# luo-ziyuan/NeRF_Signature

Measured on AMD Instinct MI355X. Metric: training rays/sec @4096 rays (hotdog, 32-bit msg), higher is better.
Workload: dtype f32 (hash gather, compositing) + fp16 MFMA with f32 accumulate (MLPs)

## Files before the change

include/nerfsig.h:

```cpp
#ifndef NERFSIG_H_
#define NERFSIG_H_

#include <stddef.h>
#include <stdint.h>

#ifdef __cplusplus
extern "C" {
#endif

#define NSIG_OK 0
#define NSIG_ERR_ARG 1
#define NSIG_ERR_LAUNCH 2

#define NSIG_TABLE_ROWS (1u << 19)
#define NSIG_BASE_LEVELS 16
#define NSIG_MAX_MESSAGE_DIM 64

typedef void *nsig_stream_t;

int nsig_abi_version(void);
const char *nsig_last_error(void);


int rm_near_far_from_aabb(const float *rays_o, const float *rays_d, const float *aabb, uint32_t N, float min_near,
// ... 164 lines not shown
int opt_adam_dense(uint32_t n, float *const *params_host, const float *const *grads_host, float *const *exp_avg_host,
                   float *const *exp_avg_sq_host, float *const *steps_host, const uint32_t *numel_host, const float *lr, float beta1,
                   float beta2, float eps, float grad_scale, float *scratch, nsig_stream_t stream);
int opt_adam_dense_host(uint32_t n, float *const *params_host, const float *const *grads_host, float *const *exp_avg_host,
                        float *const *exp_avg_sq_host, const uint32_t *numel_host, const float *step_sizes_host, const float *inv_bc2_host,
                        float beta1, float beta2, float eps, float grad_scale, nsig_stream_t stream);

int rm_composite_train_finish_fwd(const float *sigmas, const float *rgbs, const float *deltas, const int32_t *rays, uint32_t M, uint32_t N,
                                  float T_thresh, const float *nears, const float *fars, const float *bg, uint32_t bg_stride,
                                  float *weights_sum, float *depth, float *image, float *image_out, float *depth_out, nsig_stream_t stream);
int rm_composite_train_finish_bwd(const float *grad_weights_sum, const float *grad_image_out, const float *sigmas, const float *rgbs,
                                  const float *deltas, const int32_t *rays, const float *weights_sum, const float *image, const float *bg,
                                  uint32_t bg_stride, uint32_t M, uint32_t N, float T_thresh, uint32_t rays_in_order, float *grad_sigmas,
                                  float *grad_rgbs, nsig_stream_t stream);


int rm_finish_fwd(const float *image, const float *depth, const float *weights_sum, const float *nears, const float *fars, const float *bg,
                  uint32_t bg_stride, uint32_t N, float *image_out, float *depth_out, nsig_stream_t stream);
int rm_finish_bwd(const float *grad_image, const float *grad_depth, const float *depth, const float *nears, const float *fars, const float *bg,
                  uint32_t bg_stride, uint32_t N, float *grad_weights_sum, float *grad_depth_in, nsig_stream_t stream);

int loop_step_begin(float *G, uint32_t n_floats, const float *ring_dev, uint32_t slots, uint32_t width, uint32_t *counter, float *msg,
                    nsig_stream_t stream);
void *nsig_host_device_pointer(const void *pinned_host);

int wm_loss_fwd(const float *content, const float *gt, uint32_t n_content, const float *decoded, const float *message, uint32_t D, float temp,
                float lambda_w, float lambda_i, float *losses3, float *d_content, float *d_decoded, nsig_stream_t stream);
int wm_loss_bwd(const float *g_lossi, const float *g_lossw, const float *g_loss, float lambda_w, float lambda_i, const float *d_content,
                uint32_t n_content, const float *d_decoded, uint32_t D, float *grad_content, float *grad_decoded, nsig_stream_t stream);


int dec_bn_gelu_fwd(const float *x, const float *gamma, const float *beta, uint32_t N, uint32_t C, uint32_t P, float eps, float *y,
                    float *save, nsig_stream_t stream);
int dec_bn_gelu_bwd(const float *dy, const float *x, const float *gamma, const float *beta, const float *save, uint32_t N, uint32_t C,
                    uint32_t P, float *dx, float *dgamma, float *dbeta, nsig_stream_t stream);

size_t dec_workspace_bytes(uint32_t B, uint32_t Cin, uint32_t H, uint32_t W);
int dec_forward(const float *img, uint32_t input_mode, const float *mean_host, const float *std_host, const float *const *params_host,
                uint32_t B, uint32_t Cin, uint32_t H, uint32_t W, float eps, void *workspace, float *decoded, float *clamped_out,
                nsig_stream_t stream);
int dec_backward(const float *grad_decoded, const float *img, uint32_t input_mode, const float *mean_host, const float *std_host,
                 const float *const *params_host, uint32_t B, uint32_t Cin, uint32_t H, uint32_t W, void *workspace,
                 float *const *grads_host, float *grad_img, nsig_stream_t stream, nsig_stream_t weights_stream);

int dec_forward_train(const float *img, const float *mean_host, const float *std_host, const float *const *params_host, uint32_t B,
                      uint32_t Cin, uint32_t H, uint32_t W, float eps, void *workspace, float *decoded, float *clamped_out,
// ... 74 lines not shown
```

nerf_signature_amd/_native.py:

```python
import ctypes
import os

import torch

_PKG = os.path.dirname(os.path.abspath(__file__))
LIB_PATH = os.path.join(_PKG, "lib", "libnerfsig.so")

_c = ctypes
_vp, _u32, _fl, _int, _sz = _c.c_void_p, _c.c_uint32, _c.c_float, _c.c_int, _c.c_size_t

SIGNATURES = {
    "nsig_abi_version": [],
    "nsig_last_error": [],
    "nsig_host_device_pointer": [_vp],
    "rg_sample_rays": [_vp, _u32, _vp, _fl, _fl, _fl, _fl, _u32, _u32, _u32, _vp, _u32, _u32, _c.c_uint64, _vp, _vp, _vp, _vp, _vp, _vp],
    "rg_get_rays": [_vp, _fl, _fl, _fl, _fl, _u32, _u32, _vp, _u32, _u32, _vp, _vp, _vp],
    "rm_near_far_from_aabb": [_vp, _vp, _vp, _u32, _fl, _vp, _vp, _vp],
    "rm_sph_from_ray": [_vp, _vp, _fl, _u32, _vp, _vp],
    "rm_morton3D": [_vp, _u32, _vp, _vp],
    "rm_morton3D_invert": [_vp, _u32, _vp, _vp],
    "rm_packbits": [_vp, _u32, _fl, _vp, _vp],
    "rg_refresh_draw_scratch_bytes": [_u32, _u32],
    "rg_refresh_begin": [_vp, _u32, _vp],
    "rg_refresh_draw": [_vp, _vp, _u32, _u32, _vp, _vp, _c.c_uint64, _vp, _u32, _vp],
# ... 32 lines not shown
    "hg_level_lookup": [_vp, _u32, _fl, _vp, _vp, _vp],
    "opt_codebook_adam": [_vp, _vp, _vp, _vp, _u32, _fl, _fl, _fl, _vp, _vp, _fl, _vp],
    "opt_codebook_adam_sel": [_vp, _vp, _vp, _vp, _vp, _vp, _u32, _vp, _fl, _fl, _fl, _fl, _vp, _vp],
    "opt_codebook_adam_sel_next": [_vp, _vp, _vp, _vp, _vp, _vp, _u32, _vp, _fl, _fl, _fl, _fl, _vp, _vp, _vp, _vp],
    "mlp_packed_bytes": [],
    "mlp_get_precision": [],
    "mlp_set_precision": [_int],
    "mlp_get_pipelined": [],
    "mlp_set_pipelined": [_int],
    "mlp_pack_weights": [_vp, _vp, _vp, _vp],
    "hg_planes_bytes": [_u32],
    "hg_encode_planes": [_vp, _u32, _fl, _vp, _vp, _vp, _vp],
    "hg_warm_tables": [_vp, _vp, _vp, _vp],
    "hg_encode_codebook_plane": [_vp, _u32, _fl, _vp, _vp, _int, _vp, _vp],
    "field_fwd": [_vp, _vp, _u32, _fl, _vp, _vp, _vp, _vp, _vp, _vp, _vp, _vp, _int, _vp],
    "field_color_fwd": [_vp, _vp, _u32, _vp, _vp, _vp],
    "opt_adam_dense_host": [_u32, _vp, _vp, _vp, _vp, _vp, _vp, _vp, _fl, _fl, _fl, _fl, _vp],
    "opt_adam_dense": [_u32, _vp, _vp, _vp, _vp, _vp, _vp, _vp, _fl, _fl, _fl, _fl, _vp, _vp],
    "rm_composite_train_finish_fwd": [_vp, _vp, _vp, _vp, _u32, _u32, _fl, _vp, _vp, _vp, _u32, _vp, _vp, _vp, _vp, _vp, _vp],
    "rm_composite_train_finish_bwd": [_vp, _vp, _vp, _vp, _vp, _vp, _vp, _vp, _vp, _u32, _u32, _u32, _fl, _u32, _vp, _vp, _vp],
    "rm_finish_fwd": [_vp, _vp, _vp, _vp, _vp, _vp, _u32, _u32, _vp, _vp, _vp],
    "rm_finish_bwd": [_vp, _vp, _vp, _vp, _vp, _vp, _u32, _u32, _vp, _vp, _vp],
    "loop_step_begin": [_vp, _u32, _vp, _u32, _u32, _vp, _vp, _vp],
    "wm_loss_fwd": [_vp, _vp, _u32, _vp, _vp, _u32, _fl, _fl, _fl, _vp, _vp, _vp, _vp],
    "wm_loss_bwd": [_vp, _vp, _vp, _fl, _fl, _vp, _u32, _vp, _u32, _vp, _vp, _vp],
    "dec_bn_gelu_fwd": [_vp, _vp, _vp, _u32, _u32, _u32, _fl, _vp, _vp, _vp],
    "dec_bn_gelu_bwd": [_vp, _vp, _vp, _vp, _vp, _u32, _u32, _u32, _vp, _vp, _vp, _vp],
    "dec_workspace_bytes": [_u32, _u32, _u32, _u32],
    "dec_forward": [_vp, _u32, _vp, _vp, _vp, _u32, _u32, _u32, _u32, _fl, _vp, _vp, _vp, _vp],
    "dec_backward": [_vp, _vp, _u32, _vp, _vp, _vp, _u32, _u32, _u32, _u32, _vp, _vp, _vp, _vp, _vp],
    "dec_forward_train": [_vp, _vp, _vp, _vp, _u32, _u32, _u32, _u32, _fl, _vp, _vp, _vp, _u32, _vp, _vp, _vp, _fl, _fl, _vp, _vp],
    "dec_backward_train": [_vp, _vp, _vp, _vp, _vp, _u32, _u32, _u32, _u32, _vp, _vp, _vp, _u32, _vp, _vp, _vp, _vp, _vp],
    "wm_distort_draw": [_u32, _c.c_uint64, _vp, _u32, _vp, _vp, _vp],
    "wm_distort_fwd": [_vp, _u32, _u32, _u32, _u32, _u32, _vp, _vp, _vp, _vp],
    "wm_distort_bwd": [_vp, _vp, _u32, _u32, _u32, _u32, _u32, _vp, _vp, _vp, _vp],
    "wm_distort_geom_fwd": [_vp, _u32, _u32, _u32, _u32, _u32, _vp, _u32, _vp, _vp, _vp],
    "wm_distort_geom_bwd": [_vp, _vp, _u32, _u32, _u32, _u32, _u32, _vp, _u32, _vp, _vp],
    "field_fwd_trace": [_vp, _vp, _u32, _fl, _vp, _vp, _vp, _vp, _vp, _vp, _vp, _vp, _vp, _vp, _vp],
    "field_bwd_trace": [_u32, _vp, _vp, _vp, _vp, _vp, _vp, _vp, _vp, _vp, _vp, _vp, _vp, _vp],
    "hg_scatter_level": [_vp, _fl, _vp, _u32, _u32, _vp, _vp],
    "hg_scatter_binned_scratch_bytes": [_u32],
    "hg_scatter_binned": [_vp, _u32, _vp, _vp, _vp],
    "hg_scatter_levels_scratch_bytes": [_u32],
    "hg_scatter_levels": [_vp, _fl, _vp, _u32, _u32, _vp, _vp, _vp],
    "field_bwd": [_vp, _u32, _fl, _vp, _vp, _vp, _vp, _vp, _vp, _vp, _vp, _vp, _vp],
    "field_bwd_planned": [_vp, _u32, _fl, _vp, _vp, _vp, _vp, _vp, _vp, _vp, _vp],
    "hg_scatter_plan_bytes": [_u32],
    "hg_scatter_plan": [_vp, _u32, _fl, _vp, _vp],
    "hg_scatter_planned": [_vp, _u32, _vp, _vp],
    "field_fwd_trace_rows": [_vp, _vp, _u32, _vp, _fl, _vp, _vp, _vp, _vp, _vp, _vp, _vp, _vp, _vp, _vp, _vp],
    "field_fwd_trace_f16": [_vp, _vp, _u32, _vp, _fl, _vp, _vp, _vp, _vp, _vp, _vp, _vp, _vp, _vp, _vp, _vp],
    "field_bwd_trace_rows": [_u32, _vp, _vp, _vp, _vp, _vp, _vp, _vp, _vp, _vp, _vp, _vp, _vp, _vp, _vp],
    "field_wgrad_scratch_bytes": [_u32],
    "field_wgrad": [_u32, _vp, _vp, _vp, _vp, _vp, _vp, _vp, _vp, _vp, _vp, _vp, _vp, _vp, _vp, _vp],
    "field_bwd_wgrad_scratch_bytes": [_u32],
    "field_bwd_wgrad": [_u32, _vp, _vp, _vp, _vp, _vp, _vp, _vp, _vp, _vp, _vp, _vp, _vp, _vp, _vp, _vp, _vp, _vp],
    "field_bwd_wgrad_f16": [_u32, _vp, _vp, _vp, _vp, _vp, _vp, _vp, _vp, _vp, _vp, _vp, _vp, _vp, _vp, _vp, _vp, _vp],
    "rm_composite_train_mse": [_vp, _vp, _vp, _vp, _u32, _u32, _fl, _vp, _vp, _vp, _u32, _vp, _u32, _fl, _vp, _vp, _vp, _vp, _vp, _vp, _vp, _vp, _vp],
    "opt_ema_update": [_u32, _vp, _vp, _vp, _vp, _c.c_double, _vp],
    "clean_loss": [_vp, _vp, _u32, _fl, _vp, _vp, _vp, _vp, _vp, _vp, _u32, _vp, _u32, _c.c_uint64, _vp],
    "hg_levels_plan_bytes": [_u32],
    "hg_levels_plan": [_vp, _u32, _vp, _fl, _vp, _vp],
    "hg_levels_scatter": [_vp, _u32, _vp, _fl, _vp, _u32, _vp, _vp, _vp],
    "hg_levels_scatter_adam": [_vp, _u32, _vp, _fl, _vp, _u32, _vp, _vp, _vp, _vp, _vp, _vp, _fl, _fl, _fl, _fl, _vp, _vp],
}
_RESTYPES = {"nsig_last_error": _c.c_char_p, "nsig_host_device_pointer": _c.c_void_p, "rm_march_train_scratch_bytes": _sz, "mlp_packed_bytes": _sz, "hg_planes_bytes": _sz, "dec_workspace_bytes": _sz, "hg_scatter_levels_scratch_bytes": _sz, "hg_scatter_binned_scratch_bytes": _sz, "hg_scatter_plan_bytes": _sz, "field_wgrad_scratch_bytes": _sz, "field_bwd_wgrad_scratch_bytes": _sz, "hg_levels_plan_bytes": _sz, "rg_refresh_partials_bytes": _sz, "rg_refresh_draw_scratch_bytes": _sz}

_lib = None


class NativeError(RuntimeError):
    pass


def load():
    global _lib
    if _lib is not None:
        return _lib
    path = os.environ.get("NERFSIG_LIB", LIB_PATH)
    if not os.path.exists(path):
        raise NativeError(f"{path} not found: the HIP extension is required (no fallback). "
                          f"Build it with `python -m nerf_signature_amd.build`.")
    _lib = ctypes.CDLL(path)
    _lib.nsig_last_error.restype = _c.c_char_p
    return _lib


_bound = {}

# ... 71 lines not shown
```

nerf_signature_amd/csrc/hashgrid.hip:

```cpp
#include <cstdlib>
#include "hashgrid.h"

namespace nsig {

__global__ void __launch_bounds__(256) k_codebook_presum(CodebookPtrs tabs, uint32_t D, float4 *__restrict__ S) {
    const uint32_t e = blockIdx.x * blockDim.x + threadIdx.x;
    if (e >= NSIG_TABLE_ROWS / 2) return;
    float4 acc = {0.f, 0.f, 0.f, 0.f};
    uint32_t i = 0;
    for (; i + 4 <= D; i += 4) {
        const float4 a = reinterpret_cast<const float4 *>(tabs.p[i])[e];
        const float4 b = reinterpret_cast<const float4 *>(tabs.p[i + 1])[e];
        const float4 c = reinterpret_cast<const float4 *>(tabs.p[i + 2])[e];
        const float4 d = reinterpret_cast<const float4 *>(tabs.p[i + 3])[e];
        acc.x = (((acc.x + a.x) + b.x) + c.x) + d.x;
        acc.y = (((acc.y + a.y) + b.y) + c.y) + d.y;
        acc.z = (((acc.z + a.z) + b.z) + c.z) + d.z;
        acc.w = (((acc.w + a.w) + b.w) + c.w) + d.w;
    }
    for (; i < D; ++i) {
        const float4 a = reinterpret_cast<const float4 *>(tabs.p[i])[e];
        acc.x += a.x; acc.y += a.y; acc.z += a.z; acc.w += a.w;
    }
    S[e] = acc;
// ... 935 lines not shown
    const float step = *sp + 1.0f;
    *sp = step;
    scratch[i] = (float)((double)*lr / (1.0 - exp((double)step * log((double)beta1))));
    scratch[D + i] = (float)(1.0 / sqrt(1.0 - exp((double)step * log((double)beta2))));
}

typedef float nsig_f32x4 __attribute__((ext_vector_type(4)));
template <bool NT>
__device__ __forceinline__ float4 ld4(const float4 *p) {
    if (!NT) return *p;
    const nsig_f32x4 v = __builtin_nontemporal_load(reinterpret_cast<const nsig_f32x4 *>(p));
    return make_float4(v.x, v.y, v.z, v.w);
}
template <bool NT>
__device__ __forceinline__ void st4(float4 *p, const float4 &a) {
    if (!NT) {
        *p = a;
        return;
    }
    const nsig_f32x4 v = {a.x, a.y, a.z, a.w};
    __builtin_nontemporal_store(v, reinterpret_cast<nsig_f32x4 *>(p));
}

template <bool NEXT, bool NT>
__global__ void __launch_bounds__(256) k_codebook_adam_sel(const float4 *__restrict__ G, AdamPairPtrs a, const float *__restrict__ message,
                                                           const float *__restrict__ scratch, uint32_t D, float beta1, float beta2, float eps,
                                                           float grad_scale, const float *__restrict__ next_message, float4 *__restrict__ S_next) {
    const uint32_t e = blockIdx.x * blockDim.x + threadIdx.x;
    if (e >= NSIG_TABLE_ROWS / 2) return;
    float4 g = ld4<NT>(G + e);
    g.x *= grad_scale; g.y *= grad_scale; g.z *= grad_scale; g.w *= grad_scale;
    float4 acc = {0.f, 0.f, 0.f, 0.f};
    const float4 zero = {0.f, 0.f, 0.f, 0.f};
    uint32_t i = 0;
    for (; i + 2 <= D; i += 2) {
        const uint32_t j0 = 2 * i + (message[i] != 0.0f), j1 = 2 * i + 2 + (message[i + 1] != 0.0f);
        float4 *pp0 = reinterpret_cast<float4 *>(a.p[j0]) + e, *pm0 = reinterpret_cast<float4 *>(a.m[j0]) + e, *pv0 = reinterpret_cast<float4 *>(a.v[j0]) + e;
        float4 *pp1 = reinterpret_cast<float4 *>(a.p[j1]) + e, *pm1 = reinterpret_cast<float4 *>(a.m[j1]) + e, *pv1 = reinterpret_cast<float4 *>(a.v[j1]) + e;
        bool other0 = false, other1 = false;
        float4 o0 = zero, o1 = zero;
        if (NEXT) {
            other0 = (next_message[i] != 0.0f) != (message[i] != 0.0f);
            other1 = (next_message[i + 1] != 0.0f) != (message[i + 1] != 0.0f);
            if (other0) o0 = ld4<NT>(reinterpret_cast<const float4 *>(a.p[j0 ^ 1u]) + e);
            if (other1) o1 = ld4<NT>(reinterpret_cast<const float4 *>(a.p[j1 ^ 1u]) + e);
        }
        float4 p0 = ld4<NT>(pp0), m0 = ld4<NT>(pm0), v0 = ld4<NT>(pv0), p1 = ld4<NT>(pp1), m1 = ld4<NT>(pm1), v1 = ld4<NT>(pv1);
        const float ss0 = scratch[i], ib0 = scratch[D + i], ss1 = scratch[i + 1], ib1 = scratch[D + i + 1];
        adam_update(g.x, p0.x, m0.x, v0.x, beta1, beta2, eps, ss0, ib0);
        adam_update(g.y, p0.y, m0.y, v0.y, beta1, beta2, eps, ss0, ib0);
        adam_update(g.z, p0.z, m0.z, v0.z, beta1, beta2, eps, ss0, ib0);
        adam_update(g.w, p0.w, m0.w, v0.w, beta1, beta2, eps, ss0, ib0);
        adam_update(g.x, p1.x, m1.x, v1.x, beta1, beta2, eps, ss1, ib1);
        adam_update(g.y, p1.y, m1.y, v1.y, beta1, beta2, eps, ss1, ib1);
// ... 8 lines not shown
    }
    for (; i < D; ++i) {
        const uint32_t j = 2 * i + (message[i] != 0.0f);
        float4 *pp = reinterpret_cast<float4 *>(a.p[j]) + e, *pm = reinterpret_cast<float4 *>(a.m[j]) + e, *pv = reinterpret_cast<float4 *>(a.v[j]) + e;
        bool other = false;
        float4 o = zero;
        if (NEXT) {
            other = (next_message[i] != 0.0f) != (message[i] != 0.0f);
            if (other) o = ld4<NT>(reinterpret_cast<const float4 *>(a.p[j ^ 1u]) + e);
        }
        float4 p = ld4<NT>(pp), m = ld4<NT>(pm), v = ld4<NT>(pv);
        const float ss = scratch[i], ib = scratch[D + i];
        adam_update(g.x, p.x, m.x, v.x, beta1, beta2, eps, ss, ib);
        adam_update(g.y, p.y, m.y, v.y, beta1, beta2, eps, ss, ib);
        adam_update(g.z, p.z, m.z, v.z, beta1, beta2, eps, ss, ib);
        adam_update(g.w, p.w, m.w, v.w, beta1, beta2, eps, ss, ib);
        st4<NT>(pp, p); st4<NT>(pm, m); st4<NT>(pv, v);
        if (NEXT) {
            const float4 c = other ? o : p;
            acc.x += c.x; acc.y += c.y; acc.z += c.z; acc.w += c.w;
        }
    }
    if (NEXT) S_next[e] = acc;
}

}

using namespace nsig;

static int aligned16(const void *p) { return (reinterpret_cast<uintptr_t>(p) & 15) == 0; }

NSIG_EXPORT int hg_codebook_presum(const float *const *tables_host, uint32_t D, float *S, nsig_stream_t stream) {
    NSIG_REQUIRE(tables_host && S, "hg_codebook_presum: null pointer");
    NSIG_REQUIRE(D >= 1 && D <= NSIG_MAX_MESSAGE_DIM, "hg_codebook_presum: D=%u out of range [1,%d]", D, NSIG_MAX_MESSAGE_DIM);
    CodebookPtrs tabs{};
    for (uint32_t i = 0; i < D; ++i) {
        NSIG_REQUIRE(tables_host[i] && aligned16(tables_host[i]), "hg_codebook_presum: table %u is null or not 16-byte aligned", i);
        tabs.p[i] = tables_host[i];
    }
    NSIG_REQUIRE(aligned16(S), "hg_codebook_presum: S must be 16-byte aligned");
    k_codebook_presum<<<NSIG_TABLE_ROWS / 2 / 256, 256, 0, as_stream(stream)>>>(tabs, D, reinterpret_cast<float4 *>(S));
    return check_launch("hg_codebook_presum");
}

static int fill_base(const float *const *host, TablePtrs &base, const char *who) {
    NSIG_REQUIRE(host, "%s: null base table list", who);
// ... 287 lines not shown
            d.numel[k] = numel_host[j];
            d.slot[k] = (uint8_t)i;
            d.chunk0[k] = chunks;
            chunks += ceil_div(numel_host[j], wide ? kDenseChunk4 : kDenseChunk);
            ++k;
        }
        small.chunk0[n_small] = chunks_small;
        big.chunk0[n_big] = chunks_big;
        float *sc = scratch + (size_t)first * 2;
        k_adam_dense_prepare<<<1, kDenseMax, 0, st>>>(all, cnt, lr, beta1, beta2, sc);
        if (int e = check_launch("opt_adam_dense (prepare)")) return e;
        if (n_big) {
            k_adam_dense_v4<<<chunks_big, 256, 0, st>>>(big, n_big, sc, beta1, beta2, eps, grad_scale);
            if (int e = check_launch("opt_adam_dense (wide)")) return e;
        }
        if (n_small) {
            k_adam_dense<<<chunks_small, 256, 0, st>>>(small, n_small, sc, beta1, beta2, eps, grad_scale);
            if (int e = check_launch("opt_adam_dense")) return e;
        }
    }
    return NSIG_OK;
}

static size_t binned_scratch_bytes(uint32_t M, uint32_t sets) { return (size_t)sets * (sizeof(BinHeader) + (size_t)4 * M * sizeof(uint4)); }

static int reserve_owner_lds(const char *who) {
    static bool attr_set = false;
    const size_t lds = (size_t)kBinRows * 2 * sizeof(unsigned long long);
    if (!attr_set) {
        if (hipFuncSetAttribute(reinterpret_cast<const void *>(k_scatter_binned), hipFuncAttributeMaxDynamicSharedMemorySize, (int)lds) != hipSuccess) {
            set_error("%s: cannot reserve %zu bytes of LDS", who, lds);
            return NSIG_ERR_LAUNCH;
        }
        attr_set = true;
    }
    return NSIG_OK;
}

static int owner_targets_aligned(const ScatterTargets &tg, uint32_t sets, const char *who) {
    for (uint32_t i = 0; i < sets; ++i) NSIG_REQUIRE(aligned16(tg.g[i]), "%s: gradient table %u must be 16-byte aligned", who, i);
    return NSIG_OK;
}

static int launch_binned(const float *rec, uint32_t M, uint32_t sets, const ScatterTargets &tg, uint32_t replicas, void *scratch, hipStream_t st,
                         const char *who) {
    static_assert(sizeof(BinHeader) % 16 == 0 && kBinGrid == 16 * 16, "the queues follow the headers 16-byte aligned; k_bin_scan walks 16 x 16 workgroups");
// ... 209 lines not shown
```

nerf_signature_amd/optim.py:

```python
import ctypes
import math

import torch

from . import _native as nv


def fused_shared_step(optimizer, group, selected, G, grad_scale=1.0):
    beta1, beta2 = group["betas"]
    lr, eps = float(group["lr"]), float(group["eps"])
    D = len(selected)
    vp = ctypes.c_void_p * D
    pp, pm, pv, step_sizes, inv_bc2 = vp(), vp(), vp(), (ctypes.c_float * D)(), (ctypes.c_float * D)()
    handles = optimizer.__dict__.setdefault("_nsig_table_handles", {})
    state = optimizer.state
    for i, p in enumerate(selected):
        h = handles.get(id(p))
        if h is None or h[0] is not p or state.get(p) is not h[1] or h[1].get("exp_avg") is not h[2] or h[1].get("exp_avg_sq") is not h[3] or h[1].get("step") is not h[8]:
            st = optimizer.state[p]
            if len(st) == 0:
                st["step"] = torch.tensor(0.0, dtype=torch.float32)
                st["exp_avg"] = torch.zeros_like(p, memory_format=torch.preserve_format)
                st["exp_avg_sq"] = torch.zeros_like(p, memory_format=torch.preserve_format)
            for t in (p, st["exp_avg"], st["exp_avg_sq"]):
# ... 122 lines not shown
        for g in self.param_groups:
            if any(q is p for q in g["params"]):
                return g
        raise ValueError("parameter is not managed by this optimiser")

    @torch.no_grad()
    def step_shared(self, selected, G, grad_scale=1.0):
        if not selected:
            return
        fused_shared_step(self, self._group_of(selected[0]), selected, G, grad_scale)


def _prepare_device_state(opt, tables):
    for t in tables:
        st = opt.state[t]
        if len(st) == 0:
            st["step"] = torch.zeros((), dtype=torch.float32, device=t.device)
            st["exp_avg"] = torch.zeros_like(t, memory_format=torch.preserve_format)
            st["exp_avg_sq"] = torch.zeros_like(t, memory_format=torch.preserve_format)
        elif not st["step"].is_cuda:
            st["step"] = st["step"].to(t.device)


def _step_shared_sel(opt, tables, message_dev, G, lr_dev, grad_scale=1.0, next_message_dev=None, S_next=None):
    group = opt._group_of(tables[0])
    beta1, beta2 = group["betas"]
    cache = getattr(opt, "_sel_cache", None)
    if (cache is None or len(cache[0]) != len(tables) or any(a is not b for a, b in zip(cache[0], tables))
            or any(opt.state.get(t) is not st for t, st in zip(tables, cache[4]))):
        _prepare_device_state(opt, tables)
        D = len(tables) // 2
        arrays = (nv.ptr_array([t.data for t in tables]), nv.ptr_array([opt.state[t]["exp_avg"] for t in tables]),
                  nv.ptr_array([opt.state[t]["exp_avg_sq"] for t in tables]), nv.ptr_array([opt.state[t]["step"] for t in tables]))
        scratch = torch.empty(2 * D, dtype=torch.float32, device=tables[0].device)
        cache = opt._sel_cache = (list(tables), arrays, scratch, D, [opt.state[t] for t in tables])
    _, (pp, pm, pv, ps), scratch, D, _ = cache
    if next_message_dev is not None:
        if S_next is None or S_next.dtype != torch.float32 or not S_next.is_contiguous() or S_next.numel() != tables[0].numel():
            raise ValueError("step_shared_sel: S_next must be a contiguous float32 tensor of one table's size")
        nv.call("opt_codebook_adam_sel_next", nv.ptr(G), pp, pm, pv, ps, nv.ptr(message_dev), D, nv.ptr(lr_dev), float(beta1), float(beta2),
                float(group["eps"]), float(grad_scale), nv.ptr(scratch), nv.ptr(next_message_dev), nv.ptr(S_next), nv.stream())
    else:
        nv.call("opt_codebook_adam_sel", nv.ptr(G), pp, pm, pv, ps, nv.ptr(message_dev), D, nv.ptr(lr_dev), float(beta1), float(beta2),
                float(group["eps"]), float(grad_scale), nv.ptr(scratch), nv.stream())
    _bump_versions(tables)


CodebookAdam.step_shared_sel = torch.no_grad()(_step_shared_sel)


def _step_dense(opt, lr_dev, grad_scale=1.0):
    todo = []
    for group in opt.param_groups:
        for p in group["params"]:
            if p.grad is None:
                continue
            if not (p.is_cuda and p.dtype == torch.float32 and p.grad.dtype == torch.float32 and p.is_contiguous() and p.grad.is_contiguous()):
                raise NotImplementedError("step_dense handles contiguous float32 CUDA parameters")
            st = opt.state[p]
            if len(st) == 0:
                st["step"] = torch.zeros((), dtype=torch.float32, device=p.device)
                st["exp_avg"] = torch.zeros_like(p, memory_format=torch.preserve_format)
                st["exp_avg_sq"] = torch.zeros_like(p, memory_format=torch.preserve_format)
            elif not st["step"].is_cuda:
                st["step"] = st["step"].to(p.device)
            todo.append((group, p))
    if not todo:
        return
    group = todo[0][0]
    if any(g["betas"] != group["betas"] or g["eps"] != group["eps"] for g, _ in todo):
        raise NotImplementedError("step_dense expects one (betas, eps) for all dense parameters")
    ps = [p for _, p in todo]
    n = len(ps)
    scratch = getattr(opt, "_dense_scratch", None)
    if scratch is None or scratch.numel() < 64 * ((n + 31) // 32):
        scratch = opt._dense_scratch = torch.empty(64 * ((n + 31) // 32), dtype=torch.float32, device=ps[0].device)
    numel = (ctypes.c_uint32 * n)(*[p.numel() for p in ps])
    nv.call("opt_adam_dense", n, nv.ptr_array([p.data for p in ps]), nv.ptr_array([p.grad for p in ps]),
            nv.ptr_array([opt.state[p]["exp_avg"] for p in ps]), nv.ptr_array([opt.state[p]["exp_avg_sq"] for p in ps]),
            nv.ptr_array([opt.state[p]["step"] for p in ps]), numel, nv.ptr(lr_dev), float(group["betas"][0]), float(group["betas"][1]),
            float(group["eps"]), float(grad_scale), nv.ptr(scratch), nv.stream())
    _bump_versions(ps)


CodebookAdam.step_dense = torch.no_grad()(_step_dense)


def _bump_versions(tensors):
    setter = getattr(torch._C._autograd, "_unsafe_set_version_counter", None)
    if setter is not None:
        setter(list(tensors), [t._version + 1 for t in tensors])
    else:
        for t in tensors:
            t.add_(0)
```

nerf_signature_amd/trainer.py:

```python
import ctypes
import os

import numpy as np
import torch
import torch.nn.functional as F

from . import _native as nv
from . import fieldops as fo
from . import dp
from .dp import GradExchange, exchange_active, world_size
from .distortion import DistortionLayer, host_uniform, scaled_width
from .hidden_models import normalize_img, set_grad_arena, set_weights_stream


def loss_w_bce(decoded, keys, temp=10.0):
    return F.binary_cross_entropy_with_logits(decoded * temp, keys, reduction="mean")


def loss_w_mse(decoded, keys, temp=10.0):
    return torch.mean((decoded * temp - (2 * keys - 1)) ** 2)


class _WatermarkLoss(torch.autograd.Function):

    @staticmethod
    def forward(ctx, content, gt, decoded, keys, lambda_w, lambda_i, temp):
        content, gt, decoded, keys = content.contiguous(), gt.contiguous(), decoded.contiguous(), keys.contiguous()
        losses = torch.empty(3, dtype=torch.float32, device=content.device)
        d_content, d_decoded = torch.empty_like(content), torch.empty_like(decoded)
        nv.call("wm_loss_fwd", nv.ptr(content), nv.ptr(gt), content.numel(), nv.ptr(decoded), nv.ptr(keys), decoded.numel(), temp, lambda_w, lambda_i,
                nv.ptr(losses), nv.ptr(d_content), nv.ptr(d_decoded), nv.stream())
        ctx.save_for_backward(d_content, d_decoded)
        ctx.lambdas = (lambda_w, lambda_i)
        ctx.set_materialize_grads(False)
        _WatermarkLoss.stash = (d_content, d_decoded)
# ... 317 lines not shown
    def __init__(self):
        self.V, self.N = 0, 0

    def clear(self):
        self.V, self.N = 0, 0

    def update(self, preds, truths):
        p = preds.detach().cpu().numpy() if torch.is_tensor(preds) else preds
        t = truths.detach().cpu().numpy() if torch.is_tensor(truths) else truths
        self.V += -10 * np.log10(np.mean((p - t) ** 2))
        self.N += 1

    def measure(self):
        return self.V / self.N

    def report(self):
        return f"PSNR = {self.measure():.6f}"


class GraphedWatermarkLoop:

    def __init__(self, model, optimizer, render_kwargs, data, lambda_w=1.0, lambda_i=1.0, lr_lambda=None, headroom=0.0, native_dense_adam=True,
                 overlap_content=True, march_ahead=None, presum_in_adam=True, stage_in_graph=True, content_headroom=None,
                 content_sampler=None, fixed_blocks=False, distortion="none", distortion_seed=0):
        self.distortion = None if distortion in (None, "none") else (distortion if isinstance(distortion, DistortionLayer) else DistortionLayer(distortion, distortion_seed))
        self.march_ahead = overlap_content if march_ahead is None else bool(march_ahead)
        self.fixed_blocks = bool(fixed_blocks)
        self._refix_pending = False
        self._kept_key = None
        self.content_sampler = content_sampler
        self.presum_in_adam = bool(presum_in_adam)
        self.stage_in_graph = bool(stage_in_graph)
        self._s_for = None
        self.marched = None
        self._pending_content = None
        self.native_dense_adam = native_dense_adam
        self.side_stream = torch.cuda.Stream() if overlap_content else None
        self.plan_stream = self.side_stream
        self.weights_stream = self.side_stream
        self.content_backward_first = False
        if not hasattr(optimizer, "step_shared_sel"):
            raise TypeError("GraphedWatermarkLoop needs nerf_signature_amd.optim.CodebookAdam(capturable=True)")
        if not any(t.requires_grad for t in model.msg_encoder.tables()):
            raise NotImplementedError("GraphedWatermarkLoop captures the step that trains the codebook; with a frozen codebook "
                                      "(finetune_decoder=True) drive the model with WatermarkLoop")
        self.model, self.optimizer = model, optimizer
        self.render_kwargs = dict(render_kwargs)
        self.lambda_w, self.lambda_i = lambda_w, lambda_i
        self.lr_lambda, self.headroom = lr_lambda, headroom
        self.content_headroom = headroom if content_headroom is None else content_headroom
        dev = next(model.parameters()).device
        self.device = dev
        self._warm_sink = torch.zeros(1, dtype=torch.float32, device=dev)
        D = model.message_dim
        self.sink = fo.GradSink(dev, tail=sum(p.numel() for p in model.msg_decoder.parameters()))
# ... 52 lines not shown
        _prepare_device_state(self.optimizer, self.tables)
        kinds = [lambda t: t.data]
        if optimizer_state:
            dp_state = self.optimizer.state
            kinds += [lambda t, k=k: dp_state[t][k] for k in ("exp_avg", "exp_avg_sq", "step") if all(k in dp_state[t] for t in self.tables)]
        for get in kinds:
            own = torch.stack([get(t).reshape(-1) for t in self.tables[2 * b0:2 * b1]])
            every = torch.empty((world,) + tuple(own.shape), dtype=own.dtype, device=own.device)
            dp._all_gather_into(every.view(world * own.shape[0], -1), own)
            for i, t in enumerate(self.tables):
                get(t).reshape(-1).copy_(every.view(len(self.tables), -1)[i])
        from .optim import _bump_versions
        _bump_versions(self.tables)
        self.model._codebook_stale = False

    def close(self):
        self.gather_codebook()
        self.model.codebook_shard = None
        self.model.device_select = False
        self.model.point_capacity = None
        if self in getattr(self.model, "_graphed_loops", ()):
            self.model._graphed_loops.remove(self)

    def _forward_backward(self):
        if self.stage_in_graph and torch.cuda.is_current_stream_capturing():
            nv.call("loop_step_begin", nv.ptr(self.sink.G), self.sink.G.numel(), ctypes.c_void_p(self.ring_dev), len(self.msg_ring),
                    self.stage_width, nv.ptr(self.stage_counter), nv.ptr(self.msg_all), nv.stream())
        else:
            self.sink.zero_()
            if self.content_sampler is not None and torch.cuda.is_current_stream_capturing():
                self.stage_counter += 1
        if self.content_sampler is not None:
            ct = self.data["content"]
            self.content_sampler.sample_into(self.stage_counter, ct["rays_o"], ct["rays_d"], ct["images"])
        if self.distortion is not None and self.distortion.name != "scaling":
            o = self.data["watermark"]["rays_o_block"]
            self.distortion.draw_on_device(self.stage_counter, tuple(o.shape), o.device)
        prev = fo.set_plan_stream(self.plan_stream)
        try:
            out = train_step(self.model, self.data, self.msg_dev, self.render_kwargs, self.lambda_w, self.lambda_i, side_stream=self.side_stream,
                             presum_first=self.marched is not None,
                             presum_adopt=self.presum_in_adam and torch.cuda.is_current_stream_capturing(),
                             blocks_first=self.side_stream is not None and self._blocks_issued_first(),
                             content_backward_now=(self.lambda_i * dp.content_grad_scale(self.sharded)) if (self.content_backward_first and self.side_stream is not None) else None,
                             distortion=self.distortion)
        finally:
            fo.set_plan_stream(prev)
        set_weights_stream(self.weights_stream)
        set_grad_arena(self.sink.tail)
        try:
            backward_from_loss_kernel(out, dp.content_grad_scale(self.sharded), self.side_stream, self.content_backward_first)
        finally:
            set_weights_stream(None)
            set_grad_arena(None)
        join_stream(torch.cuda.current_stream(), self.side_stream)
        if self.weights_stream is not self.side_stream:
            join_stream(torch.cuda.current_stream(), self.weights_stream)
        return out

    def _optimise(self, defer_collective=False):
        post = None
        scale = 1.0 / world_size() if self.native_dense_adam else 1.0
        scale_cb = 1.0 if (self.sharded and self.native_dense_adam) else scale
        tables, msg, msg_next = self.tables, self.msg_dev, self.msg_next_dev
        if self.opt_shard is not None:
            b0, b1 = self.opt_shard
            tables, msg, msg_next = self.tables[2 * b0:2 * b1], self.msg_dev[b0:b1], self.msg_next_dev[b0:b1]
        if self.presum_in_adam:
            S = self.model._presum_cache[1]
            self.optimizer.step_shared_sel(tables, msg, self.sink.G, self.lr_dev, scale_cb, next_message_dev=msg_next, S_next=S)
            if self.opt_shard is not None:
                import torch.distributed as dist
                post = lambda: dp.collective(lambda: dist.all_reduce(S, op=dist.ReduceOp.SUM), last=True, name="all_reduce_presum")
        else:
            self.optimizer.step_shared_sel(tables, msg, self.sink.G, self.lr_dev, scale_cb)
        if self.native_dense_adam:
            self.optimizer.step_dense(self.lr_dev, scale)
        else:
            self.optimizer.step()
        if post is not None and not defer_collective:
            post()
            post = None
        return post

    def _march_ahead(self):
        kw, wm = self.render_kwargs, self.data["watermark"]
        args = (kw.get("dt_gamma", 0), kw.get("max_steps", 1024))
# ... 153 lines not shown
            self._fix_blocks()
        side = torch.cuda.Stream()
        side.wait_stream(torch.cuda.current_stream())
        with torch.cuda.stream(side):
            for _ in range(3):
                self.optimizer.zero_grad(set_to_none=True)
                self._forward_backward()
                self.exchange(self.sink.G)
                self._optimise()
        torch.cuda.current_stream().wait_stream(side)
        torch.cuda.synchronize()
        self._restore(snapshot)

        self.variants = {}
        if self.distortion is not None and self.distortion.name == "scaling":
            W = self.data["watermark"]["rays_o_block"].shape[2]
            a_factor_of = {scaled_width(W, f): f for f in (0.75 + 0.5 * i / 4096.0 for i in range(4096))}
            for w in sorted(a_factor_of):
                self.distortion.set_scaling(a_factor_of[w])
                self.variants[w] = self._capture(cap_block, cap_content)
        else:
            self.variants[None] = self._capture(cap_block, cap_content)
        self._select(next(iter(self.variants)))
        return self

    def _select(self, key):
        v = self.variants[key]
        self.segments, self.between, self.graphs, self.out = v["segments"], v["between"], v["graphs"], v["out"]
        self.capacity_rows, self.capacities = v["capacity_rows"], v["capacities"]

    def _capture(self, cap_block, cap_content):
        model = self.model
        self.optimizer.zero_grad(set_to_none=True)
        if self.march_ahead and not self.fixed_blocks:
            self._march_ahead()
        self.segments, self.between = [torch.cuda.CUDAGraph()], []

        open_capture = [True]

        def boundary(fn, last=False):
            self.segments[-1].capture_end()
            fo.forget_plan_events()
            self.model._presum_event = None
            self.between.append(fn)
            if last:
                open_capture[0] = False
# ... 98 lines not shown
```

Baseline: 4.372 million.

## Fuse codebook and dense Adam steps into one kernel with in-kernel grad zeroing

Adds a step-begin kernel that, besides staging the message, advances the Adam step counts and computes bias-correction scratch for both codebook tables and dense parameters. A single fused optimiser kernel then updates the dense tensors and codebook rows in one launch and zeroes the gradient buffer as it reads it, removing the separate memset in loop_step_begin. The intent is fewer launches and one less pass over G inside the captured graph. In exchange it adds ordering assumptions between capture and eager steps, and relies on an explicit sink zero after capture.

```diff
diff --git a/include/nerfsig.h b/include/nerfsig.h
--- a/include/nerfsig.h
+++ b/include/nerfsig.h
@@ -210,6 +210,15 @@
 
 int loop_step_begin(float *G, uint32_t n_floats, const float *ring_dev, uint32_t slots, uint32_t width, uint32_t *counter, float *msg,
                     nsig_stream_t stream);
+int loop_step_begin_adam(const float *ring_dev, uint32_t slots, uint32_t width, uint32_t *counter, float *msg, float *const *steps_host,
+                         uint32_t D, const float *lr, float beta1, float beta2, float *scratch, uint32_t n_dense,
+                         float *const *dense_steps_host, float *dense_scratch, nsig_stream_t stream);
+int opt_step_fused(float *G, float *const *params_host, float *const *exp_avg_host, float *const *exp_avg_sq_host, const float *message,
+                   uint32_t D, float beta1, float beta2, float eps, float grad_scale_cb, const float *scratch, const float *next_message,
+                   float *S_next, uint32_t n_dense, float *const *dense_params_host, const float *const *dense_grads_host,
+                   float *const *dense_exp_avg_host, float *const *dense_exp_avg_sq_host, const uint32_t *dense_numel_host,
+                   const float *dense_scratch, float grad_scale, nsig_stream_t stream);
+size_t opt_step_fused_max_dim(void);
 void *nsig_host_device_pointer(const void *pinned_host);
 
 int wm_loss_fwd(const float *content, const float *gt, uint32_t n_content, const float *decoded, const float *message, uint32_t D, float temp,
diff --git a/nerf_signature_amd/_native.py b/nerf_signature_amd/_native.py
--- a/nerf_signature_amd/_native.py
+++ b/nerf_signature_amd/_native.py
@@ -78,6 +78,9 @@
     "rm_finish_fwd": [_vp, _vp, _vp, _vp, _vp, _vp, _u32, _u32, _vp, _vp, _vp],
     "rm_finish_bwd": [_vp, _vp, _vp, _vp, _vp, _vp, _u32, _u32, _vp, _vp, _vp],
     "loop_step_begin": [_vp, _u32, _vp, _u32, _u32, _vp, _vp, _vp],
+    "loop_step_begin_adam": [_vp, _u32, _u32, _vp, _vp, _vp, _u32, _vp, _fl, _fl, _vp, _u32, _vp, _vp, _vp],
+    "opt_step_fused": [_vp, _vp, _vp, _vp, _vp, _u32, _fl, _fl, _fl, _fl, _vp, _vp, _vp, _u32, _vp, _vp, _vp, _vp, _vp, _vp, _fl, _vp],
+    "opt_step_fused_max_dim": [],
     "wm_loss_fwd": [_vp, _vp, _u32, _vp, _vp, _u32, _fl, _fl, _fl, _vp, _vp, _vp, _vp],
     "wm_loss_bwd": [_vp, _vp, _vp, _fl, _fl, _vp, _u32, _vp, _u32, _vp, _vp, _vp],
     "dec_bn_gelu_fwd": [_vp, _vp, _vp, _u32, _u32, _u32, _fl, _vp, _vp, _vp],
@@ -120,7 +123,7 @@
     "hg_levels_scatter": [_vp, _u32, _vp, _fl, _vp, _u32, _vp, _vp, _vp],
     "hg_levels_scatter_adam": [_vp, _u32, _vp, _fl, _vp, _u32, _vp, _vp, _vp, _vp, _vp, _vp, _fl, _fl, _fl, _fl, _vp, _vp],
 }
-_RESTYPES = {"nsig_last_error": _c.c_char_p, "nsig_host_device_pointer": _c.c_void_p, "rm_march_train_scratch_bytes": _sz, "mlp_packed_bytes": _sz, "hg_planes_bytes": _sz, "dec_workspace_bytes": _sz, "hg_scatter_levels_scratch_bytes": _sz, "hg_scatter_binned_scratch_bytes": _sz, "hg_scatter_plan_bytes": _sz, "field_wgrad_scratch_bytes": _sz, "field_bwd_wgrad_scratch_bytes": _sz, "hg_levels_plan_bytes": _sz, "rg_refresh_partials_bytes": _sz, "rg_refresh_draw_scratch_bytes": _sz}
+_RESTYPES = {"nsig_last_error": _c.c_char_p, "nsig_host_device_pointer": _c.c_void_p, "rm_march_train_scratch_bytes": _sz, "mlp_packed_bytes": _sz, "hg_planes_bytes": _sz, "dec_workspace_bytes": _sz, "hg_scatter_levels_scratch_bytes": _sz, "hg_scatter_binned_scratch_bytes": _sz, "hg_scatter_plan_bytes": _sz, "field_wgrad_scratch_bytes": _sz, "field_bwd_wgrad_scratch_bytes": _sz, "hg_levels_plan_bytes": _sz, "rg_refresh_partials_bytes": _sz, "rg_refresh_draw_scratch_bytes": _sz, "opt_step_fused_max_dim": _sz}
 
 _lib = None
 
diff --git a/nerf_signature_amd/csrc/hashgrid.hip b/nerf_signature_amd/csrc/hashgrid.hip
--- a/nerf_signature_amd/csrc/hashgrid.hip
+++ b/nerf_signature_amd/csrc/hashgrid.hip
@@ -981,14 +981,14 @@
     __builtin_nontemporal_store(v, reinterpret_cast<nsig_f32x4 *>(p));
 }
 
-template <bool NEXT, bool NT>
-__global__ void __launch_bounds__(256) k_codebook_adam_sel(const float4 *__restrict__ G, AdamPairPtrs a, const float *__restrict__ message,
-                                                           const float *__restrict__ scratch, uint32_t D, float beta1, float beta2, float eps,
-                                                           float grad_scale, const float *__restrict__ next_message, float4 *__restrict__ S_next) {
-    const uint32_t e = blockIdx.x * blockDim.x + threadIdx.x;
-    if (e >= NSIG_TABLE_ROWS / 2) return;
+template <bool NEXT, bool NT, bool ZERO, class Ptrs>
+__device__ __forceinline__ void codebook_adam_rows(const uint32_t e, const float4 *G, const Ptrs &a, const float *__restrict__ message,
+                                                   const float *__restrict__ scratch, uint32_t D, float beta1, float beta2, float eps,
+                                                   float grad_scale, const float *__restrict__ next_message, float4 *__restrict__ S_next,
+                                                   float4 *G_zero = nullptr) {
     float4 g = ld4<NT>(G + e);
     g.x *= grad_scale; g.y *= grad_scale; g.z *= grad_scale; g.w *= grad_scale;
+    if (ZERO) st4<NT>(G_zero + e, make_float4(0.f, 0.f, 0.f, 0.f));
     float4 acc = {0.f, 0.f, 0.f, 0.f};
     const float4 zero = {0.f, 0.f, 0.f, 0.f};
     uint32_t i = 0;
@@ -1043,6 +1043,15 @@
         }
     }
     if (NEXT) S_next[e] = acc;
+}
+
+template <bool NEXT, bool NT>
+__global__ void __launch_bounds__(256) k_codebook_adam_sel(const float4 *__restrict__ G, AdamPairPtrs a, const float *__restrict__ message,
+                                                           const float *__restrict__ scratch, uint32_t D, float beta1, float beta2, float eps,
+                                                           float grad_scale, const float *__restrict__ next_message, float4 *__restrict__ S_next) {
+    const uint32_t e = blockIdx.x * blockDim.x + threadIdx.x;
+    if (e >= NSIG_TABLE_ROWS / 2) return;
+    codebook_adam_rows<NEXT, NT, false>(e, G, a, message, scratch, D, beta1, beta2, eps, grad_scale, next_message, S_next);
 }
 
 }
@@ -1376,6 +1385,141 @@
     return NSIG_OK;
 }
 
+
+namespace nsig {
+
+constexpr uint32_t kFusedMaxDim = 48;
+struct FusedPairPtrs {
+    float *p[2 * kFusedMaxDim], *m[2 * kFusedMaxDim], *v[2 * kFusedMaxDim];
+};
+struct FusedDense {
+    float *p[kDenseMax], *m[kDenseMax], *v[kDenseMax];
+    const float *g[kDenseMax];
+    uint32_t numel[kDenseMax], chunk0[kDenseMax + 1];
+};
+struct DenseSteps {
+    float *s[kDenseMax];
+};
+
+__global__ void __launch_bounds__(256) k_step_begin_adam(const float *__restrict__ ring, uint32_t slots, uint32_t width, uint32_t *__restrict__ counter,
+                                                         float *msg, StepPtrs steps, uint32_t D, const float *lr, float *__restrict__ scratch,
+                                                         DenseSteps dsteps, uint32_t n_dense, float *__restrict__ dense_scratch, float beta1, float beta2) {
+    const uint32_t t = threadIdx.x;
+    const uint32_t slot = *counter % slots;
+    if (t < width) msg[t] = ring[(size_t)slot * width + t];
+    __syncthreads();
+    if (t == 0) *counter = *counter + 1u;
+    if (t < D) {
+        float *sp = steps.s[2 * t + (msg[t] != 0.0f)];
+        const float step = *sp + 1.0f;
+        *sp = step;
+        scratch[t] = (float)((double)*lr / (1.0 - exp((double)step * log((double)beta1))));
+        scratch[D + t] = (float)(1.0 / sqrt(1.0 - exp((double)step * log((double)beta2))));
+    } else if (t >= 128 && t - 128 < n_dense) {
+        const uint32_t i = t - 128;
+        const float step = *dsteps.s[i] + 1.0f;
+        *dsteps.s[i] = step;
+        dense_scratch[i] = (float)((double)*lr / (1.0 - exp((double)step * log((double)beta1))));
+        dense_scratch[kDenseMax + i] = (float)(1.0 / sqrt(1.0 - exp((double)step * log((double)beta2))));
+    }
+}
+
+template <bool NEXT, bool NT>
+__global__ void __launch_bounds__(256) k_optimiser_fused(float4 *G, FusedPairPtrs a, const float *__restrict__ message, const float *__restrict__ scratch,
+                                                         uint32_t D, float beta1, float beta2, float eps, float grad_scale_cb,
+                                                         const float *__restrict__ next_message, float4 *__restrict__ S_next, FusedDense d, uint32_t n_dense,
+                                                         uint32_t dense_chunks, const float *__restrict__ dense_scratch, float grad_scale) {
+    if (blockIdx.x < dense_chunks) {
+        uint32_t i = 0;
+        while (i + 1 < n_dense && blockIdx.x >= d.chunk0[i + 1]) ++i;
+        const uint32_t base = (blockIdx.x - d.chunk0[i]) * kDenseChunk;
+        const float ss = dense_scratch[i], ib = dense_scratch[kDenseMax + i];
+        float *__restrict__ pp = d.p[i], *__restrict__ pm = d.m[i], *__restrict__ pv = d.v[i];
+        const float *__restrict__ pg = d.g[i];
+#pragma unroll
+        for (int u = 0; u < 4; ++u) {
+            const uint32_t e = base + u * 256 + threadIdx.x;
+            if (e < d.numel[i]) {
+                float p = pp[e], m = pm[e], v = pv[e];
+                adam_update(pg[e] * grad_scale, p, m, v, beta1, beta2, eps, ss, ib);
+                pp[e] = p; pm[e] = m; pv[e] = v;
+            }
+        }
+        return;
+    }
+    const uint32_t e = (blockIdx.x - dense_chunks) * blockDim.x + threadIdx.x;
+    if (e >= NSIG_TABLE_ROWS / 2) return;
+    codebook_adam_rows<NEXT, NT, true>(e, G, a, message, scratch, D, beta1, beta2, eps, grad_scale_cb, next_message, S_next, G);
+}
+
+static_assert(sizeof(FusedPairPtrs) + sizeof(FusedDense) + 128 <= 4096, "k_optimiser_fused's arguments");
+
+}
+
+NSIG_EXPORT size_t opt_step_fused_max_dim(void) { return kFusedMaxDim; }
+
+NSIG_EXPORT int loop_step_begin_adam(const float *ring_dev, uint32_t slots, uint32_t width, uint32_t *counter, float *msg, float *const *steps_host,
+                                     uint32_t D, const float *lr, float beta1, float beta2, float *scratch, uint32_t n_dense,
+                                     float *const *dense_steps_host, float *dense_scratch, nsig_stream_t stream) {
+    NSIG_REQUIRE(ring_dev && counter && msg && steps_host && lr && scratch, "loop_step_begin_adam: null pointer");
+    NSIG_REQUIRE(slots >= 1 && width >= 1 && width <= 256, "loop_step_begin_adam: slots >= 1 and 1 <= width <= 256");
+    NSIG_REQUIRE(D >= 1 && D <= kFusedMaxDim, "loop_step_begin_adam: D=%u out of range [1,%u]", D, kFusedMaxDim);
+    NSIG_REQUIRE(n_dense <= (uint32_t)kDenseMax && (n_dense == 0 || (dense_steps_host && dense_scratch)), "loop_step_begin_adam: at most %d dense tensors", kDenseMax);
+    StepPtrs s{};
+    for (uint32_t j = 0; j < 2 * D; ++j) {
+        NSIG_REQUIRE(steps_host[j], "loop_step_begin_adam: step count of table %u is null", j);
+        s.s[j] = steps_host[j];
+    }
+    DenseSteps ds{};
+    for (uint32_t i = 0; i < n_dense; ++i) {
+        NSIG_REQUIRE(dense_steps_host[i], "loop_step_begin_adam: step count of dense tensor %u is null", i);
+        ds.s[i] = dense_steps_host[i];
+    }
+    k_step_begin_adam<<<1, 256, 0, as_stream(stream)>>>(ring_dev, slots, width, counter, msg, s, D, lr, scratch, ds, n_dense, dense_scratch, beta1, beta2);
+    return check_launch("loop_step_begin_adam");
+}
+
+NSIG_EXPORT int opt_step_fused(float *G, float *const *params_host, float *const *exp_avg_host, float *const *exp_avg_sq_host, const float *message,
+                               uint32_t D, float beta1, float beta2, float eps, float grad_scale_cb, const float *scratch, const float *next_message,
+                               float *S_next, uint32_t n_dense, float *const *dense_params_host, const float *const *dense_grads_host,
+                               float *const *dense_exp_avg_host, float *const *dense_exp_avg_sq_host, const uint32_t *dense_numel_host,
+                               const float *dense_scratch, float grad_scale, nsig_stream_t stream) {
+    NSIG_REQUIRE(G && params_host && exp_avg_host && exp_avg_sq_host && message && scratch, "opt_step_fused: null pointer");
+    NSIG_REQUIRE(D >= 1 && D <= kFusedMaxDim, "opt_step_fused: D=%u out of range [1,%u]", D, kFusedMaxDim);
+    NSIG_REQUIRE(aligned16(G), "opt_step_fused: G must be 16-byte aligned");
+    NSIG_REQUIRE(!next_message == !S_next && (!S_next || aligned16(S_next)), "opt_step_fused: next_message and S_next go together; S_next 16-byte aligned");
+    NSIG_REQUIRE(n_dense <= (uint32_t)kDenseMax, "opt_step_fused: at most %d dense tensors", kDenseMax);
+    NSIG_REQUIRE(n_dense == 0 || (dense_params_host && dense_grads_host && dense_exp_avg_host && dense_exp_avg_sq_host && dense_numel_host && dense_scratch),
+                 "opt_step_fused: null dense pointer");
+    FusedPairPtrs a{};
+    for (uint32_t j = 0; j < 2 * D; ++j) {
+        NSIG_REQUIRE(params_host[j] && exp_avg_host[j] && exp_avg_sq_host[j], "opt_step_fused: table %u has a null pointer", j);
+        NSIG_REQUIRE(aligned16(params_host[j]) && aligned16(exp_avg_host[j]) && aligned16(exp_avg_sq_host[j]), "opt_step_fused: table %u is not 16-byte aligned", j);
+        a.p[j] = params_host[j]; a.m[j] = exp_avg_host[j]; a.v[j] = exp_avg_sq_host[j];
+    }
+    FusedDense d{};
+    uint32_t chunks = 0;
+    for (uint32_t i = 0; i < n_dense; ++i) {
+        NSIG_REQUIRE(dense_params_host[i] && dense_grads_host[i] && dense_exp_avg_host[i] && dense_exp_avg_sq_host[i] && dense_numel_host[i] > 0,
+                     "opt_step_fused: dense tensor %u has a null pointer or no elements", i);
+        NSIG_REQUIRE(dense_numel_host[i] < kDenseBigNumel, "opt_step_fused: dense tensor %u has %u elements (at most %u)", i, dense_numel_host[i], kDenseBigNumel - 1);
+        d.p[i] = dense_params_host[i]; d.g[i] = dense_grads_host[i]; d.m[i] = dense_exp_avg_host[i]; d.v[i] = dense_exp_avg_sq_host[i];
+        d.numel[i] = dense_numel_host[i];
+        d.chunk0[i] = chunks;
+        chunks += ceil_div(dense_numel_host[i], kDenseChunk);
+    }
+    d.chunk0[n_dense] = chunks;
+    const uint32_t grid = chunks + NSIG_TABLE_ROWS / 2 / 256;
+    hipStream_t st = as_stream(stream);
+    if (next_message)
+        k_optimiser_fused<true, true><<<grid, 256, 0, st>>>(reinterpret_cast<float4 *>(G), a, message, scratch, D, beta1, beta2, eps, grad_scale_cb, next_message,
+                                                            reinterpret_cast<float4 *>(S_next), d, n_dense, chunks, dense_scratch, grad_scale);
+    else
+        k_optimiser_fused<false, false><<<grid, 256, 0, st>>>(reinterpret_cast<float4 *>(G), a, message, scratch, D, beta1, beta2, eps, grad_scale_cb, nullptr,
+                                                              nullptr, d, n_dense, chunks, dense_scratch, grad_scale);
+    return check_launch("opt_step_fused");
+}
+
 static size_t binned_scratch_bytes(uint32_t M, uint32_t sets) { return (size_t)sets * (sizeof(BinHeader) + (size_t)4 * M * sizeof(uint4)); }
 
 static int reserve_owner_lds(const char *who) {
diff --git a/nerf_signature_amd/optim.py b/nerf_signature_amd/optim.py
--- a/nerf_signature_amd/optim.py
+++ b/nerf_signature_amd/optim.py
@@ -168,9 +168,7 @@
             st["step"] = st["step"].to(t.device)
 
 
-def _step_shared_sel(opt, tables, message_dev, G, lr_dev, grad_scale=1.0, next_message_dev=None, S_next=None):
-    group = opt._group_of(tables[0])
-    beta1, beta2 = group["betas"]
+def _sel_arrays(opt, tables):
     cache = getattr(opt, "_sel_cache", None)
     if (cache is None or len(cache[0]) != len(tables) or any(a is not b for a, b in zip(cache[0], tables))
             or any(opt.state.get(t) is not st for t, st in zip(tables, cache[4]))):
@@ -180,7 +178,13 @@
                   nv.ptr_array([opt.state[t]["exp_avg_sq"] for t in tables]), nv.ptr_array([opt.state[t]["step"] for t in tables]))
         scratch = torch.empty(2 * D, dtype=torch.float32, device=tables[0].device)
         cache = opt._sel_cache = (list(tables), arrays, scratch, D, [opt.state[t] for t in tables])
-    _, (pp, pm, pv, ps), scratch, D, _ = cache
+    return cache[1], cache[2], cache[3]
+
+
+def _step_shared_sel(opt, tables, message_dev, G, lr_dev, grad_scale=1.0, next_message_dev=None, S_next=None):
+    group = opt._group_of(tables[0])
+    beta1, beta2 = group["betas"]
+    (pp, pm, pv, ps), scratch, D = _sel_arrays(opt, tables)
     if next_message_dev is not None:
         if S_next is None or S_next.dtype != torch.float32 or not S_next.is_contiguous() or S_next.numel() != tables[0].numel():
             raise ValueError("step_shared_sel: S_next must be a contiguous float32 tensor of one table's size")
@@ -195,6 +199,17 @@
 CodebookAdam.step_shared_sel = torch.no_grad()(_step_shared_sel)
 
 
+def _dense_state(opt, p):
+    st = opt.state[p]
+    if len(st) == 0:
+        st["step"] = torch.zeros((), dtype=torch.float32, device=p.device)
+        st["exp_avg"] = torch.zeros_like(p, memory_format=torch.preserve_format)
+        st["exp_avg_sq"] = torch.zeros_like(p, memory_format=torch.preserve_format)
+    elif not st["step"].is_cuda:
+        st["step"] = st["step"].to(p.device)
+    return st
+
+
 def _step_dense(opt, lr_dev, grad_scale=1.0):
     todo = []
     for group in opt.param_groups:
@@ -203,13 +218,7 @@
                 continue
             if not (p.is_cuda and p.dtype == torch.float32 and p.grad.dtype == torch.float32 and p.is_contiguous() and p.grad.is_contiguous()):
                 raise NotImplementedError("step_dense handles contiguous float32 CUDA parameters")
-            st = opt.state[p]
-            if len(st) == 0:
-                st["step"] = torch.zeros((), dtype=torch.float32, device=p.device)
-                st["exp_avg"] = torch.zeros_like(p, memory_format=torch.preserve_format)
-                st["exp_avg_sq"] = torch.zeros_like(p, memory_format=torch.preserve_format)
-            elif not st["step"].is_cuda:
-                st["step"] = st["step"].to(p.device)
+            _dense_state(opt, p)
             todo.append((group, p))
     if not todo:
         return
@@ -218,9 +227,7 @@
         raise NotImplementedError("step_dense expects one (betas, eps) for all dense parameters")
     ps = [p for _, p in todo]
     n = len(ps)
-    scratch = getattr(opt, "_dense_scratch", None)
-    if scratch is None or scratch.numel() < 64 * ((n + 31) // 32):
-        scratch = opt._dense_scratch = torch.empty(64 * ((n + 31) // 32), dtype=torch.float32, device=ps[0].device)
+    scratch = _dense_scratch(opt, n, ps[0].device)
     numel = (ctypes.c_uint32 * n)(*[p.numel() for p in ps])
     nv.call("opt_adam_dense", n, nv.ptr_array([p.data for p in ps]), nv.ptr_array([p.grad for p in ps]),
             nv.ptr_array([opt.state[p]["exp_avg"] for p in ps]), nv.ptr_array([opt.state[p]["exp_avg_sq"] for p in ps]),
@@ -230,6 +237,62 @@
 
 
 CodebookAdam.step_dense = torch.no_grad()(_step_dense)
+
+
+def _dense_scratch(opt, n, device):
+    scratch = getattr(opt, "_dense_scratch", None)
+    if scratch is None or scratch.numel() < 64 * ((n + 31) // 32):
+        scratch = opt._dense_scratch = torch.empty(64 * ((n + 31) // 32), dtype=torch.float32, device=device)
+    return scratch
+
+
+
+def fused_dense_params(opt, tables, params):
+    if params is None or len(tables) // 2 > int(nv.fn("opt_step_fused_max_dim")()) or len(params) > 32:
+        return None
+    skip = {id(t) for t in tables}
+    group0 = opt._group_of(tables[0])
+    for p in params:
+        group = opt._group_of(p)
+        if id(p) in skip or not (p.is_cuda and p.dtype == torch.float32 and p.is_contiguous() and p.numel() < 65536) \
+                or group["betas"] != group0["betas"] or group["eps"] != group0["eps"]:
+            return None
+    return list(params)
+
+
+def _step_begin_fused(opt, tables, dense, ring_dev, slots, width, counter, msg_all, lr_dev):
+    group = opt._group_of(tables[0])
+    beta1, beta2 = group["betas"]
+    (_, _, _, ps), scratch, D = _sel_arrays(opt, tables)
+    steps = nv.ptr_array([_dense_state(opt, p)["step"] for p in dense]) if dense else None
+    nv.call("loop_step_begin_adam", ctypes.c_void_p(ring_dev), slots, width, nv.ptr(counter), nv.ptr(msg_all), ps, D, nv.ptr(lr_dev), float(beta1),
+            float(beta2), nv.ptr(scratch), len(dense), steps, nv.ptr(_dense_scratch(opt, max(len(dense), 1), tables[0].device)), nv.stream())
+
+
+def _step_fused(opt, tables, dense, message_dev, G, grad_scale_cb, grad_scale, next_message_dev=None, S_next=None):
+    have = [p for g in opt.param_groups for p in g["params"] if p.grad is not None]
+    if len(have) != len(dense) or any(a is not b for a, b in zip(have, dense)):
+        raise RuntimeError("step_fused: the parameters with a gradient are not the ones whose step counts the step's head advanced")
+    group = opt._group_of(tables[0])
+    beta1, beta2 = group["betas"]
+    (pp, pm, pv, _), scratch, D = _sel_arrays(opt, tables)
+    if next_message_dev is not None and (S_next is None or S_next.dtype != torch.float32 or not S_next.is_contiguous() or S_next.numel() != tables[0].numel()):
+        raise ValueError("step_fused: S_next must be a contiguous float32 tensor of one table's size")
+    n = len(dense)
+    for p in dense:
+        if not p.grad.is_contiguous() or p.grad.dtype != torch.float32:
+            raise NotImplementedError("step_fused handles contiguous float32 gradients")
+    numel = (ctypes.c_uint32 * max(n, 1))(*[p.numel() for p in dense])
+    arr = (lambda ts: nv.ptr_array(ts)) if n else (lambda ts: None)
+    nv.call("opt_step_fused", nv.ptr(G), pp, pm, pv, nv.ptr(message_dev), D, float(beta1), float(beta2), float(group["eps"]), float(grad_scale_cb),
+            nv.ptr(scratch), nv.ptr(next_message_dev) if next_message_dev is not None else None, nv.ptr(S_next) if next_message_dev is not None else None,
+            n, arr([p.data for p in dense]), arr([p.grad for p in dense]), arr([opt.state[p]["exp_avg"] for p in dense]),
+            arr([opt.state[p]["exp_avg_sq"] for p in dense]), numel, nv.ptr(_dense_scratch(opt, max(n, 1), G.device)), float(grad_scale), nv.stream())
+    _bump_versions(list(tables) + list(dense))
+
+
+CodebookAdam.step_begin_fused = torch.no_grad()(_step_begin_fused)
+CodebookAdam.step_fused = torch.no_grad()(_step_fused)
 
 
 def _bump_versions(tensors):
diff --git a/nerf_signature_amd/trainer.py b/nerf_signature_amd/trainer.py
--- a/nerf_signature_amd/trainer.py
+++ b/nerf_signature_amd/trainer.py
@@ -11,6 +11,7 @@
 from .dp import GradExchange, exchange_active, world_size
 from .distortion import DistortionLayer, host_uniform, scaled_width
 from .hidden_models import normalize_img, set_grad_arena, set_weights_stream
+from .optim import fused_dense_params
 
 
 def loss_w_bce(decoded, keys, temp=10.0):
@@ -374,7 +375,7 @@
 
     def __init__(self, model, optimizer, render_kwargs, data, lambda_w=1.0, lambda_i=1.0, lr_lambda=None, headroom=0.0, native_dense_adam=True,
                  overlap_content=True, march_ahead=None, presum_in_adam=True, stage_in_graph=True, content_headroom=None,
-                 content_sampler=None, fixed_blocks=False, distortion="none", distortion_seed=0):
+                 content_sampler=None, fixed_blocks=False, distortion="none", distortion_seed=0, fused_step=True):
         self.distortion = None if distortion in (None, "none") else (distortion if isinstance(distortion, DistortionLayer) else DistortionLayer(distortion, distortion_seed))
         self.march_ahead = overlap_content if march_ahead is None else bool(march_ahead)
         self.fixed_blocks = bool(fixed_blocks)
@@ -383,6 +384,9 @@
         self.content_sampler = content_sampler
         self.presum_in_adam = bool(presum_in_adam)
         self.stage_in_graph = bool(stage_in_graph)
+        self.fused_step = bool(fused_step)
+        self._fused_dense = None
+        self._dense_grads = None
         self._s_for = None
         self.marched = None
         self._pending_content = None
@@ -481,8 +485,19 @@
         if self in getattr(self.model, "_graphed_loops", ()):
             self.model._graphed_loops.remove(self)
 
+    def _fused_dense_params(self):
+        if not (self.fused_step and self.stage_in_graph and self.native_dense_adam and self.opt_shard is None):
+            return None
+        return fused_dense_params(self.optimizer, self.tables, self._dense_grads)
+
     def _forward_backward(self):
-        if self.stage_in_graph and torch.cuda.is_current_stream_capturing():
+        self._fused_dense = None
+        dense = self._fused_dense_params() if self.stage_in_graph and torch.cuda.is_current_stream_capturing() else None
+        if dense is not None:
+            self._fused_dense = dense
+            self.optimizer.step_begin_fused(self.tables, self._fused_dense, self.ring_dev, len(self.msg_ring), self.stage_width, self.stage_counter,
+                                            self.msg_all, self.lr_dev)
+        elif self.stage_in_graph and torch.cuda.is_current_stream_capturing():
             nv.call("loop_step_begin", nv.ptr(self.sink.G), self.sink.G.numel(), ctypes.c_void_p(self.ring_dev), len(self.msg_ring),
                     self.stage_width, nv.ptr(self.stage_counter), nv.ptr(self.msg_all), nv.stream())
         else:
@@ -522,6 +537,14 @@
         scale = 1.0 / world_size() if self.native_dense_adam else 1.0
         scale_cb = 1.0 if (self.sharded and self.native_dense_adam) else scale
         tables, msg, msg_next = self.tables, self.msg_dev, self.msg_next_dev
+        if self._fused_dense is not None and torch.cuda.is_current_stream_capturing():
+            self.optimizer.step_fused(tables, self._fused_dense, msg, self.sink.G, scale_cb, scale,
+                                      next_message_dev=msg_next if self.presum_in_adam else None,
+                                      S_next=self.model._presum_cache[1] if self.presum_in_adam else None)
+            self._fused_dense = None
+            return None
+        if not torch.cuda.is_current_stream_capturing():
+            self._dense_grads = [p for g in self.optimizer.param_groups for p in g["params"] if p.grad is not None]
         if self.opt_shard is not None:
             b0, b1 = self.opt_shard
             tables, msg, msg_next = self.tables[2 * b0:2 * b1], self.msg_dev[b0:b1], self.msg_next_dev[b0:b1]
@@ -721,6 +744,7 @@
         else:
             self.variants[None] = self._capture(cap_block, cap_content)
         self._select(next(iter(self.variants)))
+        self.sink.zero_()
         return self
 
     def _select(self, key):
```

Measured after the change: 4.359 million (median of 6 runs). No clear change (-0.3%).
